# irenemizus/ArtStyleTransfer

Hardware: AMD Instinct MI355X
Metric: style-transfer iters/sec at L=2 (1024-px) (higher is better)
Workload: dtype f32 via f16x2 split (3 f16 MFMAs per product, f32 accumulate; the 14 large-channel conv launches of a closure as Winograd F(2,3) in that arithmetic); 1 GPU; pyramid style transfer, levels_num=3 (1536x1024+768x512+384x256), lbfgs as the reference constructs it (max_eval 1 under torch 2.10), content+noise init, seeded synthetic VGG19 weights, per-step image yield on; parallelism=1 GPU

## Files before the change

artstyletransfer_amd/_lib.py:

```python
from __future__ import annotations

import ctypes as C
import os
import subprocess
import threading

_HERE = os.path.dirname(os.path.abspath(__file__))
LIB_PATH = os.environ.get("NST_LIB") or os.path.join(_HERE, "libnst_hip.so")
CSRC = os.path.join(_HERE, "csrc")

NST_OK = 0
NST_E_STATE = -2
NST_E_UNAVAILABLE = -5
NST_VGG19_CONVS = 13
NST_MAX_LEVELS = 8
NST_LOSS_ROW = 4
NST_OPT_ADAM = 0
NST_OPT_LBFGS = 1
NST_COLOR_RGB = 0
NST_COLOR_LUMINANCE = 1
NST_POOL_MAX = 0
NST_POOL_AVG = 1

c_float_p = C.POINTER(C.c_float)
REDUCE_HOOK = C.CFUNCTYPE(None, C.c_void_p)
c_void = C.c_void_p


NST_CONV_F32, NST_CONV_BF16X3, NST_CONV_F16X2 = 0, 1, 2
CONV_MODES = {"f32": NST_CONV_F32, "bf16x3": NST_CONV_BF16X3, "f16x2": NST_CONV_F16X2}
NST_COMM_ID_BYTES = 128


class StepInfo(C.Structure):
    _fields_ = [("closures", C.c_int), ("total_closures", C.c_int), ("accepted", C.c_int),
                ("loss", C.c_float), ("lr", C.c_float), ("t", C.c_float), ("history", C.c_int)]


class Options(C.Structure):
    _fields_ = [("struct_size", C.c_int), ("conv_mode", C.c_int), ("batched", C.c_int), ("single_stream", C.c_int),
                ("use_graph", C.c_int), ("h2_band_rows", C.c_int), ("lbfgs_gram", C.c_int), ("h2_mfma16", C.c_int),
                ("h2_wg256", C.c_int), ("h2_tile_rows", C.c_int), ("gram_overlap", C.c_int), ("h2_persist", C.c_int), ("level_split", C.c_int), ("h2_winograd", C.c_int)]


SYMBOLS = {
    "nst_version": (C.c_int, []),
    "nst_last_error": (C.c_char_p, [c_void]),
    "nst_device_count": (C.c_int, [C.POINTER(C.c_int)]),
    "nst_ctx_create": (C.c_int, [C.c_int, C.POINTER(c_void), C.POINTER(c_void), C.POINTER(c_void)]),
    "nst_options_default": (None, [C.POINTER(Options)]),
    "nst_ctx_create_ex": (C.c_int, [C.c_int, C.POINTER(c_void), C.POINTER(c_void), C.POINTER(Options), C.POINTER(c_void)]),
    "nst_ctx_destroy": (None, [c_void]),
    "nst_job_configure": (C.c_int, [c_void, C.c_int, C.c_int, C.c_int]),
    "nst_job_set_taps": (C.c_int, [c_void, C.c_int, C.c_uint, C.c_int]),
    "nst_job_set_color": (C.c_int, [c_void, C.c_int]),
    "nst_job_color": (C.c_int, [c_void]),
    "nst_job_set_pooling": (C.c_int, [c_void, C.c_int]),
    "nst_job_pooling": (C.c_int, [c_void]),
    "nst_color_stats": (C.c_int, [c_void, c_void, C.c_int, C.c_int, C.POINTER(C.c_double), C.POINTER(C.c_double), c_void]),
    "nst_color_transfer_matrix": (C.c_int, [C.POINTER(C.c_double)] * 6),
    "nst_color_affine": (C.c_int, [c_void, c_void, C.c_int, C.c_int, C.POINTER(C.c_double), C.POINTER(C.c_double), c_void, c_void]),
    "nst_luminance": (C.c_int, [c_void, c_void, C.c_int, C.c_int, C.c_double, C.c_double, c_void, c_void]),
    "nst_luminance_recombine": (C.c_int, [c_void, c_void, c_void, C.c_int, C.c_int, c_void, c_void]),
    "nst_level_set_targets": (C.c_int, [c_void, C.c_int, c_void, c_void, C.c_int, C.c_int, c_void]),
    "nst_closure": (C.c_int, [c_void, c_void, C.c_float, C.c_float, C.c_float, c_void, c_void, c_void]),
    "nst_closure_levels": (C.c_int, [c_void, c_void, C.c_float, C.c_float, C.c_float, C.c_uint, c_void, c_void, c_void]),
    "nst_closure_forward": (C.c_int, [c_void, c_void, C.c_float, C.c_float, C.c_float, C.c_uint, c_void, c_void]),
    "nst_closure_backward": (C.c_int, [c_void, c_void, C.c_float, C.c_float, C.c_float, C.c_uint, c_void, c_void]),
    "nst_opt_shard_levels": (C.c_int, [c_void, C.c_uint, c_void, c_void, c_void, c_void]),
    "nst_opt_shard_levels_comm": (C.c_int, [c_void, C.c_uint, c_void]),
    "nst_opt_history": (C.c_int, [c_void, C.POINTER(C.c_int), C.POINTER(C.c_int)]),
    "nst_opt_set_closure_reuse": (C.c_int, [c_void, C.c_int]),
    "nst_opt_closure_stats": (C.c_int, [c_void, C.POINTER(C.c_long), C.POINTER(C.c_long)]),
    "nst_opt_set_lazy_backward": (C.c_int, [c_void, C.c_int]),
    "nst_opt_backward_stats": (C.c_int, [c_void, C.POINTER(C.c_long), C.POINTER(C.c_long)]),
    "nst_comm_unique_id": (C.c_int, [c_void]),
    "nst_comm_create": (C.c_int, [C.c_int, C.c_int, C.c_int, c_void, C.POINTER(c_void)]),
    "nst_comm_destroy": (None, [c_void]),
    "nst_comm_info": (C.c_int, [c_void, C.POINTER(C.c_int), C.POINTER(C.c_int), C.POINTER(C.c_long), C.POINTER(C.c_double)]),
    "nst_comm_allreduce_sum": (C.c_int, [c_void, c_void, C.c_size_t, c_void]),
    "nst_adam_step": (C.c_int, [c_void, c_void, c_void, c_void, c_void, C.c_size_t, C.c_int, C.c_double, c_void]),
    "nst_lbfgs_direction": (C.c_int, [c_void, c_void, C.POINTER(c_void), C.POINTER(c_void), C.POINTER(C.c_float), C.c_int,
                                      C.c_float, C.c_size_t, C.c_int, c_void, c_void]),
    "nst_opt_create": (C.c_int, [c_void, C.c_int, C.c_float, C.c_int, C.POINTER(c_void)]),
    "nst_opt_destroy": (None, [c_void]),
    "nst_opt_step": (C.c_int, [c_void, c_void, C.c_float, C.c_float, C.c_float, c_void, C.c_int,
                               C.POINTER(StepInfo), c_void]),
    "nst_vgg_features": (C.c_int, [c_void, c_void, C.c_int, C.c_int, C.POINTER(c_void), c_void]),
    "nst_vgg_features_backward": (C.c_int, [c_void, c_void, C.c_int, C.c_int, C.POINTER(c_void), c_void, c_void]),
    "nst_vgg_activations": (C.c_int, [c_void, c_void, C.c_int, C.c_int, C.POINTER(c_void), c_void]),
    "nst_level_activation": (C.c_int, [c_void, C.c_int, C.c_int, c_void, c_void]),
    "nst_level_image": (C.c_int, [c_void, C.c_int, c_void, c_void]),
    "nst_gram": (C.c_int, [c_void, c_void, C.c_int, C.c_int, C.c_int, C.c_int, c_void, c_void]),
    "nst_total_variation": (C.c_int, [c_void, c_void, C.c_int, C.c_int, C.c_int, c_void, c_void, c_void]),
    "nst_bicubic_half": (C.c_int, [c_void, c_void, C.c_int, C.c_int, C.c_int, c_void, c_void]),
    "nst_bicubic_half_backward": (C.c_int, [c_void, c_void, C.c_int, C.c_int, C.c_int, c_void, c_void]),
    "nst_prepare_img": (C.c_int, [c_void, c_void, C.c_int, C.c_int, c_void, c_void]),
    "nst_unprepare_img": (C.c_int, [c_void, c_void, C.c_int, C.c_int, c_void, c_void]),
    "nst_resize_bicubic": (C.c_int, [c_void, c_void, C.c_int, C.c_int, C.c_int, c_void, C.c_int, C.c_int, c_void]),
    "nst_gather_rows": (C.c_int, [c_void, c_void, c_void, C.c_size_t, C.c_int, c_void, c_void]),
    "nst_gaussian_mask_accumulate": (C.c_int, [c_void, c_void, c_void, C.c_int, C.c_int, C.c_int, C.c_double, C.c_double,
                                               C.c_double, c_void]),
    "nst_noise_blend": (C.c_int, [c_void, c_void, c_void, C.c_int, C.c_int, C.c_int, C.c_double, c_void, c_void]),
    "nst_scale": (C.c_int, [c_void, c_void, C.c_float, C.c_size_t, c_void, c_void]),
    "nst_window_sums_count": (C.c_int, [C.POINTER(C.c_size_t)]),
    "nst_window_begin": (C.c_int, [c_void, c_void, C.c_int, C.c_int, C.c_int, c_void, c_void]),
    "nst_window_end": (C.c_int, [c_void, c_void, C.c_int, C.c_int, C.c_int, C.c_float, C.c_float, C.c_float, c_void, c_void,
                                 c_void, c_void]),
    "nst_conv_mode": (C.c_int, [c_void]),
    "nst_ctx_bytes": (C.c_int, [c_void, C.POINTER(C.c_size_t)]),
    "nst_set_timing": (C.c_int, [c_void, C.c_int]),
    "nst_last_closure_ms": (C.c_int, [c_void, C.POINTER(C.c_float)]),
    "nst_last_closure_class": (C.c_int, [c_void, C.c_int, C.POINTER(C.c_float), C.POINTER(C.c_int),
                                         C.POINTER(C.c_double)]),
    "nst_dump_last_closure": (C.c_int, [c_void]),
    "nst_timing_totals": (C.c_int, [c_void, C.c_int, C.POINTER(C.c_double), C.POINTER(C.c_long),
                                    C.POINTER(C.c_double), C.c_int]),
    "nst_timing_mfma_flops": (C.c_int, [c_void, C.c_int, C.POINTER(C.c_double)]),
}

_lib = None
_lock = threading.Lock()


class NstError(RuntimeError):
    pass


# ... 37 lines not shown
```

artstyletransfer_amd/csrc/nst_opt.cpp:

```cpp
#include <hip/hip_runtime.h>

#include <algorithm>
#include <cmath>
#include <cstdlib>
#include <cstring>
#include <string>
#include <vector>

#include "../../include/nst_hip.h"
#include "nst_kernels.h"

using namespace nst;

extern "C" int nst_internal_device(const nst_ctx* ctx);
extern "C" int nst_internal_levels(const nst_ctx* ctx);
extern "C" size_t nst_internal_pixels(const nst_ctx* ctx);
extern "C" int nst_internal_channels(const nst_ctx* ctx);
extern "C" int nst_internal_fail(nst_ctx* ctx, int code, const char* msg);
extern "C" void nst_internal_poison(void* p, size_t bytes);
extern "C" int nst_internal_zero_now(void* p, size_t bytes);
extern "C" int nst_internal_lbfgs_gram(const nst_ctx* ctx);
extern "C" void nst_internal_mark(nst_ctx* ctx, void* stream);
extern "C" unsigned long long nst_internal_closure_epoch(const nst_ctx* ctx);

// ... 13 lines not shown
    int kind = 0;
    size_t n = 0;
    int channels = 3;
    int levels = 0;
    double lr = 10.0;
    int total_closures = 0;
    float* g = nullptr;
    float* losses = nullptr;
    double* scratch = nullptr;
    float* scal = nullptr;
    float* al_dev = nullptr;
    bool gram_mode = false;
    const float** vec_dev = nullptr;
    float* coef_dev = nullptr;
    double* md_scratch = nullptr;
    float* md_out = nullptr;
    unsigned char* pin2 = nullptr;
    std::vector<double> SY, YY;
    float* pinned = nullptr;
    float* m = nullptr; float* v = nullptr; int k = 0;
    int max_eval = 1;
    int history = 100;
    int n_iter = 0;
    float* d = nullptr; float* prev_g = nullptr; float* xinit = nullptr; float* q = nullptr;
    std::vector<float*> old_dirs, old_stps;
    std::vector<float> ro;
    std::vector<float*> spare;
    float* pool = nullptr;
    hipEvent_t tail = nullptr;
    hipStream_t tail_stream = nullptr;
    bool tail_set = false;
    bool want_rows = false;
    bool H_is_one = true; float H_diag = 1.f;
    bool t_is_float = true;
    double t = 0.0;
    bool have_prev = false;
    unsigned level_mask = 0xFFFFFFFFu;
    nst_reduce_hook hook = nullptr;
    void* hook_user = nullptr;
    float* own_g = nullptr; float* own_losses = nullptr;
    nst_comm* comm = nullptr;
    float* pack = nullptr;
    size_t pack_floats = 0;
    std::vector<float> loss_rows;
    bool reuse = true;
    ClosureMemo memo;
    long served = 0;
    bool lazy = true;
    bool fwd_pending = false;
    bool no_halves = false;
    unsigned long long no_halves_epoch = 0;
    long forward_only = 0;
    long skipped = 0;
};

namespace {

#define OHIP(o, expr)                                                                                \
    do {                                                                                             \
        hipError_t _e = (expr);                                                                      \
        if (_e != hipSuccess)                                                                        \
            return nst_internal_fail((o)->ctx, NST_E_HIP, (std::string(#expr) + ": " + hipGetErrorString(_e)).c_str()); \
    } while (0)
#define OCHK(expr)                   \
    do {                             \
        int _r = (expr);             \
        if (_r != NST_OK) return _r; \
    } while (0)

int oalloc(nst_opt* o, float** p, size_t n) {
    hipError_t e = hipMalloc(reinterpret_cast<void**>(p), n * sizeof(float));
    if (e != hipSuccess) return nst_internal_fail(o->ctx, NST_E_NOMEM, "hipMalloc failed in optimiser");
    nst_internal_poison(*p, n * sizeof(float));
    return NST_OK;
}

struct GradStats {
    bool want_abs = false;
    const float* dot_with = nullptr;
    float gmax = 0.f, gsum = 0.f, gdot = 0.f;
};

int eval_closure(nst_opt* o, const float* x, float cw, float sw, float tvw, hipStream_t s, float* loss_out,
                 GradStats* gs = nullptr, bool forward_only = false) {
    o->lr *= 0.999;
    o->fwd_pending = false;
    if (forward_only && !(o->no_halves && o->no_halves_epoch == nst_internal_closure_epoch(o->ctx))) {
        const int rc = nst_closure_forward(o->ctx, x, cw, sw, tvw, o->level_mask, o->losses, s);
        if (rc == NST_OK) { o->fwd_pending = true; o->forward_only += 1; }
        else if (rc != NST_E_UNAVAILABLE) return rc;
        o->no_halves = rc == NST_E_UNAVAILABLE;
        o->no_halves_epoch = nst_internal_closure_epoch(o->ctx);
    }
    if (!o->fwd_pending) OCHK(nst_closure_levels(o->ctx, x, cw, sw, tvw, o->level_mask, o->g, o->losses, s));
    if (o->comm) OCHK(nst_comm_allreduce_sum(o->comm, o->pack, o->pack_floats, s));
    else if (o->hook) o->hook(o->hook_user);
    const size_t row = (size_t)NST_LOSS_ROW * o->levels + 1;
    const size_t off = o->loss_rows.size();
    o->loss_rows.resize(off + row);
    float* hrow = o->pinned + 8;
    OHIP(o, hipMemcpyAsync(hrow, o->losses, row * sizeof(float), hipMemcpyDeviceToHost, s));
    float* r = o->pinned;
    if (gs && gs->want_abs) OHIP(o, launch_absmax_abssum(o->g, o->n, o->scratch, o->scal, s));
    if (gs && gs->dot_with) OHIP(o, launch_dot(o->g, gs->dot_with, o->n, o->scratch, o->scal + 2, s));
    if (gs) OHIP(o, hipMemcpyAsync(r, o->scal, 3 * sizeof(float), hipMemcpyDeviceToHost, s));
    OHIP(o, hipStreamSynchronize(s));
    if (o->comm) {
        float total = hrow[0];
        for (int l = 1; l < o->levels; ++l) total = total + hrow[(size_t)NST_LOSS_ROW * l];
        hrow[row - 1] = total;
    }
    std::memcpy(o->loss_rows.data() + off, hrow, row * sizeof(float));
    if (gs) { gs->gmax = r[0]; gs->gsum = r[1]; gs->gdot = r[2]; }
    o->total_closures += 1;
    *loss_out = o->loss_rows[off + row - 1];
    return NST_OK;
}

int dot(nst_opt* o, const float* a, const float* b, hipStream_t s, float* out) {
    OHIP(o, launch_dot(a, b, o->n, o->scratch, o->scal, s));
    OHIP(o, hipMemcpyAsync(o->pinned, o->scal, sizeof(float), hipMemcpyDeviceToHost, s));
    OHIP(o, hipStreamSynchronize(s));
    *out = o->pinned[0];
    return NST_OK;
}
int dot2(nst_opt* o, const float* a0, const float* b0, const float* a1, const float* b1, hipStream_t s, float* out0,
         float* out1) {
    float* r = o->pinned;
    OHIP(o, launch_dot(a0, b0, o->n, o->scratch, o->scal, s));
    OHIP(o, launch_dot(a1, b1, o->n, o->scratch, o->scal + 1, s));
    OHIP(o, hipMemcpyAsync(r, o->scal, 2 * sizeof(float), hipMemcpyDeviceToHost, s));
    OHIP(o, hipStreamSynchronize(s));
    *out0 = r[0]; *out1 = r[1];
    return NST_OK;
}
int dot_and_absstats(nst_opt* o, const float* g, const float* d, hipStream_t s, float* gtd, float* mx, float* sum) {
    float* r = o->pinned;
    OHIP(o, launch_absmax_abssum(d, o->n, o->scratch, o->scal, s));
    OHIP(o, launch_dot(g, d, o->n, o->scratch, o->scal + 2, s));
    OHIP(o, hipMemcpyAsync(r, o->scal, 3 * sizeof(float), hipMemcpyDeviceToHost, s));
    OHIP(o, hipStreamSynchronize(s));
    *mx = r[0]; *sum = r[1]; *gtd = r[2];
    return NST_OK;
}
int absstats(nst_opt* o, const float* a, hipStream_t s, float* mx, float* sum) {
    float* r = o->pinned;
    OHIP(o, launch_absmax_abssum(a, o->n, o->scratch, o->scal, s));
    OHIP(o, hipMemcpyAsync(r, o->scal, 2 * sizeof(float), hipMemcpyDeviceToHost, s));
    OHIP(o, hipStreamSynchronize(s));
    *mx = r[0]; *sum = r[1];
    return NST_OK;
}

double cubic_interpolate(double x1, double f1, double g1, double x2, double f2, double g2, bool has_bounds,
                         double lo, double hi) {
    double xmin = has_bounds ? lo : std::min(x1, x2);
    double xmax = has_bounds ? hi : std::max(x1, x2);
    const double d1 = g1 + g2 - 3 * (f1 - f2) / (x1 - x2);
    const double d2sq = d1 * d1 - g1 * g2;
    if (d2sq >= 0) {
        const double d2 = std::sqrt(d2sq);
        double min_pos;
        if (x1 <= x2) min_pos = x2 - (x2 - x1) * ((g2 + d2 - d1) / (g2 - g1 + 2 * d2));
        else min_pos = x1 - (x1 - x2) * ((g1 + d2 - d1) / (g1 - g2 + 2 * d2));
        return std::min(std::max(min_pos, xmin), xmax);
    }
    return (xmin + xmax) / 2.0;
}

struct LsResult { double t; float f; int evals; double last_t; };

bool lazy_applies(const nst_opt* o);

int strong_wolfe(nst_opt* o, float* x, double t, float f, float gtd, float d_norm, int max_ls, float cw, float sw,
                 float tvw, hipStream_t s, LsResult* res) {
    const double c1 = 1e-4, c2 = 0.9, tol_change = 1e-9;
    double last_t = t;
    const bool lazy = lazy_applies(o);
    auto eval_at = [&](double tt, int ls_after, float* f_new, float* gtd_new) -> int {
        last_t = tt;
        OHIP(o, launch_add_scaled(o->xinit, (float)tt, o->d, x, o->n, s));
        if (lazy && ls_after == max_ls) {
            *gtd_new = 0.f;
            return eval_closure(o, x, cw, sw, tvw, s, f_new, nullptr, true);
        }
        GradStats gs;
        gs.dot_with = o->d;
        OCHK(eval_closure(o, x, cw, sw, tvw, s, f_new, &gs));
        *gtd_new = gs.gdot;
        return NST_OK;
    };
    float f_new, gtd_new;
    OCHK(eval_at(t, 0, &f_new, &gtd_new));
    int evals = 1;
    double t_prev = 0; float f_prev = f; float gtd_prev = gtd;
    bool done = false;
    int ls_iter = 0;
    double br[2] = {0, 0}; float br_f[2] = {0, 0}; float br_gtd[2] = {0, 0};
    int nbr = 0;
    while (ls_iter < max_ls) {
        if (f_new > (float)(f + (float)(c1 * t) * gtd) || (ls_iter > 1 && f_new >= f_prev)) {
            br[0] = t_prev; br[1] = t; br_f[0] = f_prev; br_f[1] = f_new; br_gtd[0] = gtd_prev; br_gtd[1] = gtd_new; nbr = 2;
            break;
        }
        if (std::fabs(gtd_new) <= -(float)c2 * gtd) {
            br[0] = t; br_f[0] = f_new; br_gtd[0] = gtd_new; nbr = 1; done = true;
            break;
        }
        if (gtd_new >= 0) {
            br[0] = t_prev; br[1] = t; br_f[0] = f_prev; br_f[1] = f_new; br_gtd[0] = gtd_prev; br_gtd[1] = gtd_new; nbr = 2;
            break;
        }
        const double min_step = t + 0.01 * (t - t_prev);
        const double max_step = t * 10;
        const double tmp = t;
        t = cubic_interpolate(t_prev, f_prev, gtd_prev, t, f_new, gtd_new, true, min_step, max_step);
        t_prev = tmp; f_prev = f_new; gtd_prev = gtd_new;
        OCHK(eval_at(t, ls_iter + 1, &f_new, &gtd_new));
        evals += 1;
        ls_iter += 1;
    }
    if (ls_iter == max_ls && nbr == 0) {
        br[0] = 0; br[1] = t; br_f[0] = f; br_f[1] = f_new; br_gtd[0] = gtd; br_gtd[1] = gtd_new; nbr = 2;
    }
    bool insuf = false;
    int low = (br_f[0] <= br_f[nbr - 1]) ? 0 : 1, high = 1 - low;
    if (nbr == 1) { low = 0; high = 0; }
    while (!done && ls_iter < max_ls) {
        if (std::fabs(br[1] - br[0]) * d_norm < tol_change) break;
        t = cubic_interpolate(br[0], br_f[0], br_gtd[0], br[1], br_f[1], br_gtd[1], false, 0, 0);
        const double bmax = std::max(br[0], br[1]), bmin = std::min(br[0], br[1]);
        const double eps = 0.1 * (bmax - bmin);
        if (std::min(bmax - t, t - bmin) < eps) {
            if (insuf || t >= bmax || t <= bmin) {
                t = (std::fabs(t - bmax) < std::fabs(t - bmin)) ? bmax - eps : bmin + eps;
                insuf = false;
            } else {
                insuf = true;
            }
        } else {
            insuf = false;
        }
        OCHK(eval_at(t, ls_iter + 1, &f_new, &gtd_new));
        evals += 1;
        ls_iter += 1;
        if (f_new > (float)(f + (float)(c1 * t) * gtd) || f_new >= br_f[low]) {
// ... 27 lines not shown
        for (int j = 0; j < i; ++j) v += (al[j] - be[j]) * SYm[(size_t)j * ld + i];
        be[i] = (double)ro[i] * v;
    }
    for (int j = 0; j < m; ++j) { coef[j] = (float)(-(double)Hd * al[j]); coef[m + j] = (float)(al[j] - be[j]); }
}

int gram_direction(nst_opt* o, bool new_pair, hipStream_t s) {
    const int m = (int)o->old_dirs.size();
    const int Hh = o->history;
    const float Hd = o->H_is_one ? 1.f : o->H_diag;
    OHIP(o, launch_scale_copy(-1.f, o->g, o->q, o->n, s));
    if (m == 0) {
        OHIP(o, launch_scale_copy(Hd, o->q, o->d, o->n, s));
        return NST_OK;
    }
    const float** hp = reinterpret_cast<const float**>(o->pin2);
    float* hcoef = reinterpret_cast<float*>(o->pin2 + 2 * (size_t)Hh * sizeof(float*));
    float* hres = hcoef + 2 * (size_t)Hh;
    for (int j = 0; j < m; ++j) { hp[j] = o->old_dirs[j]; hp[m + j] = o->old_stps[j]; }
    OHIP(o, hipMemcpyAsync(o->vec_dev, hp, 2 * (size_t)m * sizeof(float*), hipMemcpyHostToDevice, s));
    const float* a = new_pair ? o->old_stps[m - 1] : o->q;
    const float* b = new_pair ? o->old_dirs[m - 1] : o->q;
    OHIP(o, launch_multi_dot(o->vec_dev, 2 * m, a, b, o->q, o->n, o->md_scratch, o->md_out, s));
    OHIP(o, hipMemcpyAsync(hres, o->md_out, 2 * (size_t)m * 3 * sizeof(float), hipMemcpyDeviceToHost, s));
    OHIP(o, hipStreamSynchronize(s));
    auto SY = [&](int i, int j) -> double& { return o->SY[(size_t)i * Hh + j]; };
    auto YY = [&](int i, int j) -> double& { return o->YY[(size_t)i * Hh + j]; };
    if (new_pair) {
        const int k = m - 1;
        for (int j = 0; j < m; ++j) {
            SY(k, j) = hres[(size_t)j * 3 + 0];
            YY(k, j) = YY(j, k) = hres[(size_t)j * 3 + 1];
            SY(j, k) = hres[(size_t)(m + j) * 3 + 1];
        }
    }
    std::vector<double> sq(m), yq(m);
    for (int i = 0; i < m; ++i) { sq[i] = hres[(size_t)(m + i) * 3 + 2]; yq[i] = hres[(size_t)i * 3 + 2]; }
    direction_coefficients(m, Hh, o->SY.data(), o->YY.data(), o->ro.data(), Hd, sq.data(), yq.data(), hcoef);
    OHIP(o, hipMemcpyAsync(o->coef_dev, hcoef, 2 * (size_t)m * sizeof(float), hipMemcpyHostToDevice, s));
    OHIP(o, launch_multi_axpy(o->vec_dev, o->coef_dev, 2 * m, o->q, Hd, o->d, o->n, s));
    return NST_OK;
}

bool memo_applies(const nst_opt* o) {
    const unsigned all = o->levels >= 32 ? 0xFFFFFFFFu : (1u << o->levels) - 1u;
    return o->reuse && !o->comm && !o->hook && (o->level_mask & all) == all;
}

bool lazy_applies(const nst_opt* o) {
    const unsigned all = o->levels >= 32 ? 0xFFFFFFFFu : (1u << o->levels) - 1u;
    return o->lazy && o->kind == NST_OPT_LBFGS && !o->comm && !o->hook && (o->level_mask & all) == all;
}

int serve_closure(nst_opt* o, const float* x, float cw, float sw, float tvw, unsigned long long epoch, hipStream_t s,
                  bool* served) {
    *served = false;
    ClosureMemo& M = o->memo;
    const float w[3] = {cw, sw, tvw};
    if (std::memcmp(M.w, w, sizeof(w)) != 0 || M.epoch != epoch) return NST_OK;
    float* r = o->pinned;
    OHIP(o, launch_count_diff(x, o->xinit, o->n, o->scratch, o->scal + 3, s));
    if (!M.have_abs) OHIP(o, launch_absmax_abssum(o->g, o->n, o->scratch, o->scal, s));
    OHIP(o, hipMemcpyAsync(r, o->scal, 4 * sizeof(float), hipMemcpyDeviceToHost, s));
    OHIP(o, hipStreamSynchronize(s));
    unsigned diff;
    std::memcpy(&diff, r + 3, sizeof(diff));
    if (diff != 0) return NST_OK;
    if (!M.have_abs) { M.gmax = r[0]; M.gsum = r[1]; M.have_abs = true; }
    o->lr *= 0.999;
    o->loss_rows.insert(o->loss_rows.end(), M.row.begin(), M.row.end());
    o->total_closures += 1;
    o->served += 1;
    *served = true;
    return NST_OK;
}

int form_direction(nst_opt* o, double lr, float gsum, hipStream_t s, double* t, float* gtd, float* d_norm, float* d_sum) {
    if (o->n_iter == 1) {
        OHIP(o, launch_scale_copy(-1.f, o->g, o->d, o->n, s));
        for (float* p : o->old_dirs) o->spare.push_back(p);
        for (float* p : o->old_stps) o->spare.push_back(p);
        o->old_dirs.clear(); o->old_stps.clear(); o->ro.clear();
        o->H_is_one = true; o->H_diag = 1.f;
        if (o->gram_mode) { std::fill(o->SY.begin(), o->SY.end(), 0.0); std::fill(o->YY.begin(), o->YY.end(), 0.0); }
    } else {
        float* y; float* st;
        auto take = [&](float** p) -> int {
            if (o->spare.empty()) return nst_internal_fail(o->ctx, NST_E_STATE, "L-BFGS history pool exhausted");
            *p = o->spare.back(); o->spare.pop_back();
            return NST_OK;
        };
        OCHK(take(&y)); OCHK(take(&st));
        OHIP(o, launch_sub(o->g, o->prev_g, y, o->n, s));
        OHIP(o, launch_scale_copy((float)o->t, o->d, st, o->n, s));
        float ys, yy;
        OCHK(dot2(o, y, st, y, y, s, &ys, &yy));
        bool new_pair = false;
        if (ys > 1e-10f) {
            if ((int)o->old_dirs.size() == o->history) {
                o->spare.push_back(o->old_dirs.front()); o->spare.push_back(o->old_stps.front());
                o->old_dirs.erase(o->old_dirs.begin()); o->old_stps.erase(o->old_stps.begin()); o->ro.erase(o->ro.begin());
                if (o->gram_mode) {
                    const int Hh = o->history;
                    for (int i = 0; i + 1 < Hh; ++i)
                        for (int j = 0; j + 1 < Hh; ++j) {
                            o->SY[(size_t)i * Hh + j] = o->SY[(size_t)(i + 1) * Hh + j + 1];
                            o->YY[(size_t)i * Hh + j] = o->YY[(size_t)(i + 1) * Hh + j + 1];
                        }
                }
            }
            o->old_dirs.push_back(y); o->old_stps.push_back(st); o->ro.push_back(1.0f / ys);
            o->H_diag = ys / yy; o->H_is_one = false;
            new_pair = true;
        } else {
            o->spare.push_back(y); o->spare.push_back(st);
        }
        if (o->gram_mode) {
            OCHK(gram_direction(o, new_pair, s));
        } else {
        const int num_old = (int)o->old_dirs.size();
        double* pp[2] = {o->scratch, o->scratch + RED_BLOCKS};
        int cur = 0;
        OHIP(o, launch_scale_copy(-1.f, o->g, o->q, o->n, s));
        if (num_old > 0) OHIP(o, launch_dot_partial(o->old_stps[num_old - 1], o->q, o->n, pp[cur], s));
        for (int i = num_old - 1; i >= 0; --i) {
            OHIP(o, launch_lbfgs_pair(pp[cur], o->ro[i], o->al_dev + i, 0, o->old_dirs[i], o->q,
                                      i > 0 ? o->old_stps[i - 1] : nullptr, o->n, pp[cur ^ 1], s));
            cur ^= 1;
        }
        OHIP(o, launch_scale_copy(o->H_is_one ? 1.f : o->H_diag, o->q, o->d, o->n, s));
        if (num_old > 0) OHIP(o, launch_dot_partial(o->old_dirs[0], o->d, o->n, pp[cur], s));
        for (int i = 0; i < num_old; ++i) {
            OHIP(o, launch_lbfgs_pair(pp[cur], o->ro[i], o->al_dev + i, 1, o->old_stps[i], o->d,
                                      i + 1 < num_old ? o->old_dirs[i + 1] : nullptr, o->n, pp[cur ^ 1], s));
            cur ^= 1;
        }
        }
    }
    OHIP(o, launch_copy(o->g, o->prev_g, o->n, s));
    o->have_prev = true;
    if (o->n_iter == 1) {
        const float inv = 1.0f / gsum;
        *t = (inv < 1.0f) ? (double)(inv * (float)lr) : lr;
    } else {
        *t = lr;
    }
    OCHK(dot_and_absstats(o, o->g, o->d, s, gtd, d_norm, d_sum));
    return NST_OK;
}

int lbfgs_step(nst_opt* o, float* x, float cw, float sw, float tvw, hipStream_t s, nst_step_info* info) {
    const double lr = o->lr;
    const bool memo_on = memo_applies(o);
    const unsigned long long epoch = nst_internal_closure_epoch(o->ctx);
    ClosureMemo& M = o->memo;
    const bool memo_valid = M.valid;
    M.valid = false;
    bool served = false;
    if (memo_on && memo_valid) OCHK(serve_closure(o, x, cw, sw, tvw, epoch, s, &served));
    const bool reuse_dir = served && M.have_dir;
    float loss, gmax, gsum;
    if (served) {
        loss = M.row.back(); gmax = M.gmax; gsum = M.gsum;
    } else {
        GradStats g0;
        g0.want_abs = true;
        OCHK(eval_closure(o, x, cw, sw, tvw, s, &loss, &g0));
        gmax = g0.gmax; gsum = g0.gsum;
    }
    info->loss = loss;
    const size_t row = (size_t)NST_LOSS_ROW * o->levels + 1;
    auto remember = [&](bool have_dir, bool have_abs, const float* prow, bool copy_x) -> int {
        if (copy_x) OHIP(o, launch_copy(x, o->xinit, o->n, s));
        M.have_dir = have_dir; M.have_abs = have_abs;
        M.gmax = gmax; M.gsum = gsum;
        M.w[0] = cw; M.w[1] = sw; M.w[2] = tvw;
        M.epoch = epoch;
        M.row.assign(prow, prow + row);
        M.valid = true;
        return NST_OK;
    };
    if (gmax <= 1e-7f) {
        info->accepted = 0; info->t = 0.f;
        if (memo_on) OCHK(remember(false, true, o->loss_rows.data(), !served));
        return NST_OK;
    }
    o->n_iter += 1;
    double t;
    float gtd, d_norm, d_sum;
    if (reuse_dir) {
        gtd = M.gtd; d_norm = M.d_norm; d_sum = M.d_sum;
        t = lr;
    } else {
        OCHK(form_direction(o, lr, gsum, s, &t, &gtd, &d_norm, &d_sum));
    }
    info->accepted = 0; info->t = 0.f;
    const bool ran_ls = !(gtd > -1e-9f);
    bool moved = false, g_at_x = false;
    if (ran_ls) {
        if (!served) OHIP(o, launch_copy(x, o->xinit, o->n, s));
        LsResult r;
        OCHK(strong_wolfe(o, x, t, loss, gtd, d_norm, o->max_eval - 1, cw, sw, tvw, s, &r));
        t = r.t;
        if (t != 0.0) OHIP(o, launch_add_scaled(o->xinit, (float)t, o->d, x, o->n, s));
        else OHIP(o, launch_copy(o->xinit, x, o->n, s));
        info->accepted = (t != 0.0) ? 1 : 0;
        info->t = (float)t;
        moved = t != 0.0;
        g_at_x = moved && r.last_t == t;
        if (o->fwd_pending) {
            if (g_at_x) OCHK(nst_closure_backward(o->ctx, x, cw, sw, tvw, o->level_mask, o->g, s));
            else o->skipped += 1;
            o->fwd_pending = false;
        }
    }
    o->t = t;
    if (memo_on) {
        if (!moved) {
            M.gtd = gtd; M.d_norm = d_norm; M.d_sum = d_sum;
            OCHK(remember(true, true, o->loss_rows.data(), !served && !ran_ls));
        } else if (g_at_x) {
            OCHK(remember(false, false, o->loss_rows.data() + o->loss_rows.size() - row, true));
        }
    }
    return NST_OK;
}

}

extern "C" {

int nst_opt_create(nst_ctx* ctx, int kind, float lr_start, int lbfgs_max_eval, nst_opt** out) {
    if (!ctx || !out) return nst_internal_fail(ctx, NST_E_ARG, "null argument");
    if (kind != NST_OPT_ADAM && kind != NST_OPT_LBFGS) return nst_internal_fail(ctx, NST_E_ARG, "Unknown optimizer");
    if (nst_internal_levels(ctx) < 1) return nst_internal_fail(ctx, NST_E_STATE, "nst_job_configure has not been called");
    if (hipSetDevice(nst_internal_device(ctx)) != hipSuccess) return nst_internal_fail(ctx, NST_E_HIP, "hipSetDevice failed");
    nst_opt* o = new (std::nothrow) nst_opt();
    if (!o) return nst_internal_fail(ctx, NST_E_NOMEM, "out of host memory");
    o->ctx = ctx; o->kind = kind; o->lr = (double)lr_start;
    o->levels = nst_internal_levels(ctx);
    o->channels = nst_internal_channels(ctx);
    o->n = (size_t)o->channels * nst_internal_pixels(ctx);
    o->max_eval = lbfgs_max_eval < 1 ? 1 : lbfgs_max_eval;
    const char* reuse_env = std::getenv("NST_CLOSURE_REUSE");
    o->reuse = !(reuse_env && reuse_env[0] && std::atoi(reuse_env) == 0);
    const char* lazy_env = std::getenv("NST_LAZY_BACKWARD");
    o->lazy = !(lazy_env && lazy_env[0] && std::atoi(lazy_env) == 0);
    const size_t row = (size_t)NST_LOSS_ROW * o->levels + 1;
    const size_t n_pad = (o->n + 63) & ~(size_t)63;
    o->pack_floats = n_pad + row;
    int r = oalloc(o, &o->pack, o->pack_floats);
    if (r == NST_OK && nst_internal_zero_now(o->pack, o->pack_floats * sizeof(float))) r = NST_E_HIP;
    o->g = o->own_g = o->pack;
    o->losses = o->own_losses = o->pack ? o->pack + n_pad : nullptr;
    if (r == NST_OK) r = oalloc(o, &o->scal, 4);
    if (r == NST_OK && hipEventCreateWithFlags(&o->tail, hipEventDisableTiming) != hipSuccess) r = NST_E_HIP;
    if (r == NST_OK && kind == NST_OPT_LBFGS) r = oalloc(o, &o->al_dev, (size_t)o->history);
    if (r == NST_OK && kind == NST_OPT_LBFGS && nst_internal_lbfgs_gram(ctx)) {
        const size_t H2 = 2 * (size_t)o->history;
        o->gram_mode = true;
        o->SY.assign((size_t)o->history * o->history, 0.0);
        o->YY.assign((size_t)o->history * o->history, 0.0);
        if (hipMalloc(reinterpret_cast<void**>(&o->vec_dev), H2 * sizeof(float*)) != hipSuccess ||
            hipMalloc(reinterpret_cast<void**>(&o->md_scratch), (size_t)multi_dot_blocks(o->n) * H2 * 3 * sizeof(double)) != hipSuccess ||
            hipHostMalloc(reinterpret_cast<void**>(&o->pin2), H2 * (sizeof(float*) + 4 * sizeof(float)), hipHostMallocDefault) != hipSuccess)
            r = NST_E_NOMEM;
        if (r == NST_OK) r = oalloc(o, &o->coef_dev, H2);
        if (r == NST_OK) r = oalloc(o, &o->md_out, H2 * 3);
    }
    if (r == NST_OK && hipHostMalloc(reinterpret_cast<void**>(&o->pinned), (8 + (size_t)NST_LOSS_ROW * NST_MAX_LEVELS + 1) * sizeof(float), hipHostMallocDefault) != hipSuccess) r = NST_E_NOMEM;
    if (r == NST_OK && hipMalloc(reinterpret_cast<void**>(&o->scratch), 2 * RED_BLOCKS * sizeof(double)) != hipSuccess) r = NST_E_NOMEM;
    if (r == NST_OK && kind == NST_OPT_ADAM) {
        r = oalloc(o, &o->m, o->n);
        if (r == NST_OK) r = oalloc(o, &o->v, o->n);
        if (r == NST_OK && (nst_internal_zero_now(o->m, o->n * 4) || nst_internal_zero_now(o->v, o->n * 4))) r = NST_E_HIP;
    }
    if (r == NST_OK && kind == NST_OPT_LBFGS) {
        r = oalloc(o, &o->d, o->n);
        if (r == NST_OK) r = oalloc(o, &o->prev_g, o->n);
        if (r == NST_OK) r = oalloc(o, &o->xinit, o->n);
        if (r == NST_OK) r = oalloc(o, &o->q, o->n);
        const size_t nvec = 2 * (size_t)o->history + 2;
        if (r == NST_OK) r = oalloc(o, &o->pool, nvec * n_pad);
        if (r == NST_OK) {
            o->spare.reserve(nvec);
            for (size_t i = nvec; i-- > 0;) o->spare.push_back(o->pool + i * n_pad);
        }
    }
    if (r != NST_OK) { nst_opt_destroy(o); return nst_internal_fail(ctx, r, "optimiser allocation failed"); }
    *out = o;
    return NST_OK;
}

void nst_opt_destroy(nst_opt* o) {
    if (!o) return;
    (void)hipSetDevice(nst_internal_device(o->ctx));
    if (o->tail) { (void)hipEventSynchronize(o->tail); (void)hipEventDestroy(o->tail); }
    float* ptrs[] = {o->pack, o->scal, o->al_dev, o->m, o->v, o->d, o->prev_g, o->xinit, o->q, o->pool};
    for (float* p : ptrs) if (p) (void)hipFree(p);
    if (o->scratch) (void)hipFree(o->scratch);
    if (o->pinned) (void)hipHostFree(o->pinned);
    if (o->pin2) (void)hipHostFree(o->pin2);
    if (o->vec_dev) (void)hipFree(o->vec_dev);
    if (o->md_scratch) (void)hipFree(o->md_scratch);
    if (o->coef_dev) (void)hipFree(o->coef_dev);
    if (o->md_out) (void)hipFree(o->md_out);
    delete o;
}

int nst_opt_shard_levels(nst_opt* o, unsigned level_mask, float* grad, float* losses, nst_reduce_hook hook, void* user) {
    if (!o) return nst_internal_fail(nullptr, NST_E_ARG, "null optimiser");
    if ((hook != nullptr) != (grad != nullptr && losses != nullptr))
        return nst_internal_fail(o->ctx, NST_E_ARG, "a reduce hook needs caller-owned grad and losses buffers (and vice versa)");
    o->level_mask = level_mask;
    o->hook = hook; o->hook_user = user;
    o->comm = nullptr;
    o->memo.valid = false;
    o->g = grad ? grad : o->own_g;
    o->losses = losses ? losses : o->own_losses;
    return NST_OK;
}

int nst_opt_shard_levels_comm(nst_opt* o, unsigned level_mask, nst_comm* comm) {
    if (!o) return nst_internal_fail(nullptr, NST_E_ARG, "null optimiser");
    o->level_mask = comm ? level_mask : 0xFFFFFFFFu;
    o->hook = nullptr; o->hook_user = nullptr;
    o->comm = comm;
    o->g = o->own_g; o->losses = o->own_losses;
    o->memo.valid = false;
    return NST_OK;
}

int nst_opt_history(const nst_opt* o, int* pairs, int* n_iter) {
    if (!o) return nst_internal_fail(nullptr, NST_E_ARG, "null optimiser");
    if (pairs) *pairs = (int)o->old_dirs.size();
    if (n_iter) *n_iter = o->kind == NST_OPT_ADAM ? o->k : o->n_iter;
    return NST_OK;
}

int nst_opt_set_closure_reuse(nst_opt* o, int enabled) {
    if (!o) return nst_internal_fail(nullptr, NST_E_ARG, "null optimiser");
    o->reuse = enabled != 0;
    o->memo.valid = false;
    return NST_OK;
}

int nst_opt_closure_stats(const nst_opt* o, long* evaluated, long* served) {
    if (!o) return nst_internal_fail(nullptr, NST_E_ARG, "null optimiser");
    if (evaluated) *evaluated = (long)o->total_closures - o->served;
    if (served) *served = o->served;
    return NST_OK;
}

int nst_opt_set_lazy_backward(nst_opt* o, int enabled) {
    if (!o) return nst_internal_fail(nullptr, NST_E_ARG, "null optimiser");
    o->lazy = enabled != 0;
    return NST_OK;
}

int nst_opt_backward_stats(const nst_opt* o, long* forward_only, long* skipped) {
    if (!o) return nst_internal_fail(nullptr, NST_E_ARG, "null optimiser");
    if (forward_only) *forward_only = o->forward_only;
    if (skipped) *skipped = o->skipped;
    return NST_OK;
}

static int adam_update(nst_ctx* ctx, float* x, const float* g, float* m, float* v, size_t n, int k, double lr, hipStream_t s,
                       float* step_size_out) {
    const double bc1 = 1.0 - std::pow(0.9, k);
    const double bc2 = 1.0 - std::pow(0.999, k);
    const double step_size = lr / bc1;
    const hipError_t e = launch_adam(x, g, m, v, n, 0.999f, (float)(1.0 - 0.9), (float)(1.0 - 0.999), 1e-8f, (float)step_size,
                                     (float)std::sqrt(bc2), s);
    if (e != hipSuccess) return nst_internal_fail(ctx, NST_E_HIP, hipGetErrorString(e));
    if (step_size_out) *step_size_out = (float)step_size;
    return NST_OK;
}

int nst_adam_step(nst_ctx* ctx, float* x, const float* g, float* m, float* v, size_t n, int k, double lr, void* stream) {
    if (!ctx || !x || !g || !m || !v || k < 1) return nst_internal_fail(ctx, NST_E_ARG, "bad argument");
    if (hipSetDevice(nst_internal_device(ctx)) != hipSuccess) return nst_internal_fail(ctx, NST_E_HIP, "hipSetDevice failed");
    return adam_update(ctx, x, g, m, v, n, k, lr, static_cast<hipStream_t>(stream), nullptr);
}

int nst_lbfgs_direction(nst_ctx* ctx, const float* g, const float* const* y, const float* const* sv, const float* ro, int m,
                        float h_diag, size_t n, int form, float* d, void* stream) {
    if (!ctx || !g || !d || m < 0 || (m > 0 && (!y || !sv || !ro)) || (form != 0 && form != 1))
        return nst_internal_fail(ctx, NST_E_ARG, "bad argument");
    if (hipSetDevice(nst_internal_device(ctx)) != hipSuccess) return nst_internal_fail(ctx, NST_E_HIP, "hipSetDevice failed");
    hipStream_t s = static_cast<hipStream_t>(stream);
    nst_opt tmp;
    tmp.ctx = ctx;
    nst_opt* o = &tmp;
    float* q = nullptr; float* al_dev = nullptr; float* coef_dev = nullptr; float* md_out = nullptr;
    double* scratch = nullptr; double* md_scratch = nullptr; const float** vec_dev = nullptr;
    auto cleanup = [&]() {
        (void)hipStreamSynchronize(s);
        for (void* p : {(void*)q, (void*)al_dev, (void*)coef_dev, (void*)md_out, (void*)scratch, (void*)md_scratch, (void*)vec_dev})
            if (p) (void)hipFree(p);
    };
    auto body = [&]() -> int {
        OHIP(o, hipMalloc(reinterpret_cast<void**>(&q), n * sizeof(float)));
        OHIP(o, launch_scale_copy(-1.f, g, q, n, s));
        if (m == 0) { OHIP(o, launch_scale_copy(h_diag, q, d, n, s)); return NST_OK; }
        if (form == 1) {
            OHIP(o, hipMalloc(reinterpret_cast<void**>(&al_dev), (size_t)m * sizeof(float)));
            OHIP(o, hipMalloc(reinterpret_cast<void**>(&scratch), 2 * RED_BLOCKS * sizeof(double)));
            double* pp[2] = {scratch, scratch + RED_BLOCKS};
            int cur = 0;
// ... 96 lines not shown
```

artstyletransfer_amd/engine.py:

```python
from __future__ import annotations

import ctypes as C
from typing import List, Optional, Sequence, Tuple

import numpy as np
import torch

from . import _lib
from . import taps as _taps
from .pooling_modes import check_pooling
from ._lib import NST_LOSS_ROW, NstError, StepInfo

TAP_CHANNELS = (64, 128, 256, 512, 512, 512)
TAP_SCALE = (0, 1, 2, 3, 3, 4)
DEFAULT_TAPS = (_taps.DEFAULT_CONTENT_INDEX, _taps.DEFAULT_STYLE_INDICES, True)


def _ptr(t: Optional[torch.Tensor]):
    return C.c_void_p(t.data_ptr()) if t is not None else C.c_void_p(0)


def _stream(device) -> C.c_void_p:
    return C.c_void_p(torch.cuda.current_stream(device).cuda_stream)

# ... 466 lines not shown

class PixelOptimizer:

    def __init__(self, engine: StyleEngine, name: str, lr_start: float = 10.0, lbfgs_max_eval: int = 1):
        if name == "adam":
            kind = _lib.NST_OPT_ADAM
        elif name == "lbfgs":
            kind = _lib.NST_OPT_LBFGS
        else:
            raise RuntimeError("Unknown optimizer")
        self.engine = engine
        self.name = name
        h = C.c_void_p()
        _lib.check(engine.ctx, engine.lib.nst_opt_create(engine.ctx, kind, lr_start, lbfgs_max_eval, C.byref(h)),
                   "nst_opt_create")
        self.h = h
        self.channels = engine.channels
        self.row = NST_LOSS_ROW * engine.levels + 1
        self.cap = 32 if name == "lbfgs" else 1
        self._rows = np.zeros((self.cap, self.row), dtype=np.float32)

    def shard_levels_comm(self, comm: "Communicator") -> None:
        from . import sharding
        e = self.engine
        self._comm = comm
        _lib.check(e.ctx, e.lib.nst_opt_shard_levels_comm(self.h, sharding.level_mask(e.levels, comm.rank, comm.world),
                                                          comm.h), "nst_opt_shard_levels_comm")

    def history(self):
        p, n = C.c_int(), C.c_int()
        _lib.check(self.engine.ctx, self.engine.lib.nst_opt_history(self.h, C.byref(p), C.byref(n)), "nst_opt_history")
        return p.value, n.value

    def set_closure_reuse(self, enabled: bool) -> None:
        _lib.check(self.engine.ctx, self.engine.lib.nst_opt_set_closure_reuse(self.h, int(bool(enabled))),
                   "nst_opt_set_closure_reuse")

    def closure_stats(self):
        ev, sv = C.c_long(), C.c_long()
        _lib.check(self.engine.ctx, self.engine.lib.nst_opt_closure_stats(self.h, C.byref(ev), C.byref(sv)),
                   "nst_opt_closure_stats")
        return ev.value, sv.value

    def set_lazy_backward(self, enabled: bool) -> None:
        _lib.check(self.engine.ctx, self.engine.lib.nst_opt_set_lazy_backward(self.h, int(bool(enabled))),
                   "nst_opt_set_lazy_backward")

    def backward_stats(self):
        fo, sk = C.c_long(), C.c_long()
        _lib.check(self.engine.ctx, self.engine.lib.nst_opt_backward_stats(self.h, C.byref(fo), C.byref(sk)),
                   "nst_opt_backward_stats")
        return fo.value, sk.value

    def shard_levels(self, rank: int, world: int, dist_mod=None, group=None) -> None:
        from . import sharding
        e = self.engine
        H, W = e.shape
        self._g = torch.zeros((1, self.channels, H, W), dtype=torch.float32, device=e.device)
        self._l = torch.zeros(self.row, dtype=torch.float32, device=e.device)

        def hook(_user):
            sharding.allreduce_closure(self._g, self._l, dist_mod, group)

        self._hook = _lib.REDUCE_HOOK(hook)
        _lib.check(e.ctx, e.lib.nst_opt_shard_levels(self.h, sharding.level_mask(e.levels, rank, world),
                                                     _ptr(self._g), _ptr(self._l), self._hook, None),
                   "nst_opt_shard_levels")

    def shard_stripes(self, rank: int, world: int, weights, content_t, style_t,
                      dist_mod=None, group=None, comm: "Communicator" = None) -> None:
        from . import sharding
        if comm is not None:
            rank, world = comm.rank, comm.world
        elif dist_mod is None:
            import torch.distributed as dist_mod
        contents = list(content_t) if isinstance(content_t, (list, tuple)) else [content_t]
        styles = list(style_t) if isinstance(style_t, (list, tuple)) else [style_t]
        e = self.engine
        if e.channels != 3:
            raise NstError("the stripe closure implements RGB only (set_color('rgb'))")
        H, W = e.shape
        nstriped = min(len(contents), len(styles), e.levels)
        plans, stripes = [], []
        for l in range(nstriped):
            plan = sharding.StripePlan(H >> l, world, rank)
            st = StyleEngine(weights, e.device)
            st.configure(1, plan.ext_rows, W >> l)
            st.set_targets(0, plan.cut(contents[l]), styles[l].contiguous())
            plans.append(plan)
            stripes.append(st)
        self._stripes, self._plans = stripes, plans
        self._stripe, self._plan = stripes[0], plans[0]
        n = 3 * H * W
        self._pack = torch.zeros(n + self.row, dtype=torch.float32, device=e.device)
        self._g = self._pack[:n].view(1, 3, H, W)
        self._l = self._pack[n:]
        count = stripes[0].window_sums_count()
        sums_all = torch.empty(nstriped * count, dtype=torch.float32, device=e.device)
        mask = 0
        for l in sharding.deal_levels(range(nstriped, e.levels), world)[rank]:
            mask |= 1 << l

        def hook(_user):
            x, (cw, sw, tvw) = self._x, self._w
            imgs, cuts = [x], []
            for l in range(nstriped):
# ... 97 lines not shown
```

include/nst_hip.h:

```cpp
#ifndef NST_HIP_H
#define NST_HIP_H

#include <stddef.h>
#include <stdint.h>

#ifdef __cplusplus
extern "C" {
#endif

#define NST_OK 0
#define NST_E_ARG (-1)
#define NST_E_STATE (-2)
#define NST_E_HIP (-3)
#define NST_E_NOMEM (-4)
#define NST_E_UNAVAILABLE (-5)

#define NST_VGG19_CONVS 13
#define NST_MAX_LEVELS 8
#define NST_LOSS_ROW 4

typedef struct nst_ctx nst_ctx;
typedef struct nst_opt nst_opt;
typedef struct nst_comm nst_comm;

// ... 37 lines not shown
int nst_job_color(const nst_ctx* ctx);

#define NST_POOL_MAX 0
#define NST_POOL_AVG 1
int nst_job_set_pooling(nst_ctx* ctx, int mode);
int nst_job_pooling(const nst_ctx* ctx);

int nst_level_set_targets(nst_ctx* ctx, int level, const float* content, const float* style,
                          int hs, int ws, void* stream);

int nst_closure(nst_ctx* ctx, const float* x, float content_weight, float style_weight,
                float tv_weight, float* grad, float* losses, void* stream);

int nst_closure_levels(nst_ctx* ctx, const float* x, float content_weight, float style_weight,
                       float tv_weight, unsigned level_mask, float* grad, float* losses, void* stream);

int nst_closure_forward(nst_ctx* ctx, const float* x, float content_weight, float style_weight, float tv_weight,
                        unsigned level_mask, float* losses, void* stream);
int nst_closure_backward(nst_ctx* ctx, const float* x, float content_weight, float style_weight, float tv_weight,
                         unsigned level_mask, float* grad, void* stream);

#define NST_OPT_ADAM 0
#define NST_OPT_LBFGS 1
int nst_opt_create(nst_ctx* ctx, int kind, float lr_start, int lbfgs_max_eval, nst_opt** out);
void nst_opt_destroy(nst_opt* opt);

typedef struct nst_step_info {
    int closures;
    int total_closures;
    int accepted;
    float loss;
    float lr;
    float t;
    int history;
} nst_step_info;

int nst_opt_step(nst_opt* opt, float* x, float content_weight, float style_weight, float tv_weight,
                 float* losses_host, int closures_capacity, nst_step_info* info, void* stream);

typedef void (*nst_reduce_hook)(void* user);
int nst_opt_shard_levels(nst_opt* opt, unsigned level_mask, float* grad, float* losses, nst_reduce_hook hook,
                         void* user);

int nst_opt_shard_levels_comm(nst_opt* opt, unsigned level_mask, nst_comm* comm);

int nst_opt_history(const nst_opt* opt, int* pairs, int* n_iter);

int nst_opt_set_closure_reuse(nst_opt* opt, int enabled);
int nst_opt_closure_stats(const nst_opt* opt, long* evaluated, long* served);

int nst_opt_set_lazy_backward(nst_opt* opt, int enabled);
int nst_opt_backward_stats(const nst_opt* opt, long* forward_only, long* skipped);

#define NST_COMM_ID_BYTES 128
int nst_comm_unique_id(void* id);
int nst_comm_create(int device, int rank, int world, const void* id, nst_comm** out);
void nst_comm_destroy(nst_comm* comm);
int nst_comm_info(const nst_comm* comm, int* rank, int* world, long* calls, double* bytes);
int nst_comm_allreduce_sum(nst_comm* comm, float* buf, size_t n, void* stream);

int nst_adam_step(nst_ctx* ctx, float* x, const float* g, float* m, float* v, size_t n, int k, double lr, void* stream);
int nst_lbfgs_direction(nst_ctx* ctx, const float* g, const float* const* y, const float* const* s, const float* ro, int m,
                        float h_diag, size_t n, int form, float* d, void* stream);


int nst_vgg_features(nst_ctx* ctx, const float* x, int h, int w, float* const* outs, void* stream);
int nst_vgg_activations(nst_ctx* ctx, const float* x, int h, int w, float* const* outs, void* stream);
int nst_vgg_features_backward(nst_ctx* ctx, const float* x, int h, int w, const float* const* gouts,
                              float* gx, void* stream);
int nst_level_activation(nst_ctx* ctx, int level, int layer, float* out, void* stream);
int nst_level_image(nst_ctx* ctx, int level, float* out, void* stream);
int nst_gram(nst_ctx* ctx, const float* f, int C, int h, int w, int normalize, float* gram, void* stream);
int nst_total_variation(nst_ctx* ctx, const float* y, int C, int h, int w, float* value, float* grad,
                        void* stream);
int nst_bicubic_half(nst_ctx* ctx, const float* x, int C, int h, int w, float* y, void* stream);
int nst_bicubic_half_backward(nst_ctx* ctx, const float* gy, int C, int h, int w, float* gx, void* stream);
int nst_prepare_img(nst_ctx* ctx, const float* hwc, int h, int w, float* chw, void* stream);
int nst_unprepare_img(nst_ctx* ctx, const float* chw, int h, int w, float* hwc, void* stream);


int nst_resize_bicubic(nst_ctx* ctx, const float* src, int h, int w, int channels, float* dst, int nh, int nw, void* stream);
int nst_gather_rows(nst_ctx* ctx, const float* src, const long long* perm, size_t rows, int channels, float* dst, void* stream);
int nst_gaussian_mask_accumulate(nst_ctx* ctx, float* acc, const float* src, int h, int w, int channels, double central,
                                 double peripheral, double dispersion, void* stream);
int nst_noise_blend(nst_ctx* ctx, const float* content, const float* noise, int h, int w, int channels, double noise_factor,
                    float* out, void* stream);
int nst_scale(nst_ctx* ctx, const float* src, float alpha, size_t n, float* dst, void* stream);

int nst_color_stats(nst_ctx* ctx, const float* hwc, int h, int w, double* mean, double* cov, void* stream);
int nst_color_transfer_matrix(const double* mean_c, const double* cov_c, const double* mean_s, const double* cov_s, double* A,
                              double* b);
int nst_color_affine(nst_ctx* ctx, const float* src, int h, int w, const double* A, const double* b, float* dst, void* stream);
int nst_luminance(nst_ctx* ctx, const float* hwc, int h, int w, double alpha, double beta, float* out, void* stream);
int nst_luminance_recombine(nst_ctx* ctx, const float* u, const float* content, int h, int w, float* out, void* stream);

int nst_window_sums_count(size_t* count);
int nst_window_begin(nst_ctx* ctx, const float* xs, int row0, int rows, int H0, float* sums, void* stream);
int nst_window_end(nst_ctx* ctx, const float* xs, int row0, int rows, int H0, float content_weight, float style_weight,
                   float tv_weight, float* sums, float* gxs, float* losses, void* stream);

int nst_conv_mode(const nst_ctx* ctx);

int nst_ctx_bytes(const nst_ctx* ctx, size_t* bytes);

int nst_set_timing(nst_ctx* ctx, int enabled);
int nst_last_closure_ms(nst_ctx* ctx, float* ms);
// ... 10 lines not shown
```

Before: 445.8 iters/s.

## Speculatively evaluate the L-BFGS trial point before confirming closure memo equality

When the closure memo applies and max_eval is 1, the optimiser launches the forward pass at xinit + lr*d straight away, together with the equality check against the incoming x. It then reads back the losses and the diff flag in one synchronisation. If the inputs match, the memoised closure and the trial forward are both booked, and the line search reuses that loss instead of evaluating again. The intent is to remove a separate host sync and readback between serving the memo and the trial forward. If the check fails, the speculative forward is wasted work, and the bookkeeping of lr and loss rows becomes more intricate.

```diff
diff --git a/artstyletransfer_amd/_lib.py b/artstyletransfer_amd/_lib.py
--- a/artstyletransfer_amd/_lib.py
+++ b/artstyletransfer_amd/_lib.py
@@ -74,6 +74,8 @@
     "nst_opt_closure_stats": (C.c_int, [c_void, C.POINTER(C.c_long), C.POINTER(C.c_long)]),
     "nst_opt_set_lazy_backward": (C.c_int, [c_void, C.c_int]),
     "nst_opt_backward_stats": (C.c_int, [c_void, C.POINTER(C.c_long), C.POINTER(C.c_long)]),
+    "nst_opt_set_trial_speculation": (C.c_int, [c_void, C.c_int]),
+    "nst_opt_speculation_stats": (C.c_int, [c_void, C.POINTER(C.c_long), C.POINTER(C.c_long)]),
     "nst_comm_unique_id": (C.c_int, [c_void]),
     "nst_comm_create": (C.c_int, [C.c_int, C.c_int, C.c_int, c_void, C.POINTER(c_void)]),
     "nst_comm_destroy": (None, [c_void]),
diff --git a/artstyletransfer_amd/csrc/nst_opt.cpp b/artstyletransfer_amd/csrc/nst_opt.cpp
--- a/artstyletransfer_amd/csrc/nst_opt.cpp
+++ b/artstyletransfer_amd/csrc/nst_opt.cpp
@@ -89,6 +89,9 @@
     unsigned long long no_halves_epoch = 0;
     long forward_only = 0;
     long skipped = 0;
+    bool speculate = true;
+    long spec_launched = 0;
+    long spec_discarded = 0;
 };
 
 namespace {
@@ -118,6 +121,13 @@
     float gmax = 0.f, gsum = 0.f, gdot = 0.f;
 };
 
+void book_row(nst_opt* o, const float* hrow, float* loss_out) {
+    const size_t row = (size_t)NST_LOSS_ROW * o->levels + 1;
+    o->loss_rows.insert(o->loss_rows.end(), hrow, hrow + row);
+    o->total_closures += 1;
+    *loss_out = o->loss_rows.back();
+}
+
 int eval_closure(nst_opt* o, const float* x, float cw, float sw, float tvw, hipStream_t s, float* loss_out,
                  GradStats* gs = nullptr, bool forward_only = false) {
     o->lr *= 0.999;
@@ -133,8 +143,6 @@
     if (o->comm) OCHK(nst_comm_allreduce_sum(o->comm, o->pack, o->pack_floats, s));
     else if (o->hook) o->hook(o->hook_user);
     const size_t row = (size_t)NST_LOSS_ROW * o->levels + 1;
-    const size_t off = o->loss_rows.size();
-    o->loss_rows.resize(off + row);
     float* hrow = o->pinned + 8;
     OHIP(o, hipMemcpyAsync(hrow, o->losses, row * sizeof(float), hipMemcpyDeviceToHost, s));
     float* r = o->pinned;
@@ -147,10 +155,8 @@
         for (int l = 1; l < o->levels; ++l) total = total + hrow[(size_t)NST_LOSS_ROW * l];
         hrow[row - 1] = total;
     }
-    std::memcpy(o->loss_rows.data() + off, hrow, row * sizeof(float));
     if (gs) { gs->gmax = r[0]; gs->gsum = r[1]; gs->gdot = r[2]; }
-    o->total_closures += 1;
-    *loss_out = o->loss_rows[off + row - 1];
+    book_row(o, hrow, loss_out);
     return NST_OK;
 }
 
@@ -210,7 +216,7 @@
 bool lazy_applies(const nst_opt* o);
 
 int strong_wolfe(nst_opt* o, float* x, double t, float f, float gtd, float d_norm, int max_ls, float cw, float sw,
-                 float tvw, hipStream_t s, LsResult* res) {
+                 float tvw, hipStream_t s, LsResult* res, const float* pre_f = nullptr) {
     const double c1 = 1e-4, c2 = 0.9, tol_change = 1e-9;
     double last_t = t;
     const bool lazy = lazy_applies(o);
@@ -228,7 +234,8 @@
         return NST_OK;
     };
     float f_new, gtd_new;
-    OCHK(eval_at(t, 0, &f_new, &gtd_new));
+    if (pre_f) { f_new = *pre_f; gtd_new = 0.f; }
+    else OCHK(eval_at(t, 0, &f_new, &gtd_new));
     int evals = 1;
     double t_prev = 0; float f_prev = f; float gtd_prev = gtd;
     bool done = false;
@@ -362,6 +369,13 @@
     return o->lazy && o->kind == NST_OPT_LBFGS && !o->comm && !o->hook && (o->level_mask & all) == all;
 }
 
+void book_served(nst_opt* o) {
+    o->lr *= 0.999;
+    o->loss_rows.insert(o->loss_rows.end(), o->memo.row.begin(), o->memo.row.end());
+    o->total_closures += 1;
+    o->served += 1;
+}
+
 int serve_closure(nst_opt* o, const float* x, float cw, float sw, float tvw, unsigned long long epoch, hipStream_t s,
                   bool* served) {
     *served = false;
@@ -377,11 +391,41 @@
     std::memcpy(&diff, r + 3, sizeof(diff));
     if (diff != 0) return NST_OK;
     if (!M.have_abs) { M.gmax = r[0]; M.gsum = r[1]; M.have_abs = true; }
+    book_served(o);
+    *served = true;
+    return NST_OK;
+}
+
+bool speculation_applies(const nst_opt* o, float cw, float sw, float tvw, unsigned long long epoch) {
+    const ClosureMemo& M = o->memo;
+    const float w[3] = {cw, sw, tvw};
+    return o->speculate && lazy_applies(o) && o->max_eval - 1 == 0 && M.have_dir && M.have_abs &&
+           std::memcmp(M.w, w, sizeof(w)) == 0 && M.epoch == epoch && M.gmax > 1e-7f && !(M.gtd > -1e-9f) &&
+           !(o->no_halves && o->no_halves_epoch == epoch);
+}
+int speculative_trial(nst_opt* o, const float* x, double t, float cw, float sw, float tvw, unsigned long long epoch,
+                      hipStream_t s, bool* launched, bool* equal, float* f_trial) {
+    *launched = false; *equal = false;
+    const size_t row = (size_t)NST_LOSS_ROW * o->levels + 1;
+    OHIP(o, launch_add_scaled(o->xinit, (float)t, o->d, o->q, o->n, s));
+    const int rc = nst_closure_forward(o->ctx, o->q, cw, sw, tvw, o->level_mask, o->losses, s);
+    if (rc == NST_E_UNAVAILABLE) { o->no_halves = true; o->no_halves_epoch = epoch; return NST_OK; }
+    OCHK(rc);
+    *launched = true;
+    o->spec_launched += 1;
+    OHIP(o, launch_count_diff(x, o->xinit, o->n, o->scratch, o->losses + row, s));
+    float* hrow = o->pinned + 8;
+    OHIP(o, hipMemcpyAsync(hrow, o->losses, (row + 1) * sizeof(float), hipMemcpyDeviceToHost, s));
+    OHIP(o, hipStreamSynchronize(s));
+    unsigned diff;
+    std::memcpy(&diff, hrow + row, sizeof(diff));
+    if (diff != 0) { o->spec_discarded += 1; return NST_OK; }
+    *equal = true;
+    book_served(o);
     o->lr *= 0.999;
-    o->loss_rows.insert(o->loss_rows.end(), M.row.begin(), M.row.end());
-    o->total_closures += 1;
-    o->served += 1;
-    *served = true;
+    o->fwd_pending = true;
+    o->forward_only += 1;
+    book_row(o, hrow, f_trial);
     return NST_OK;
 }
 
@@ -467,7 +511,13 @@
     const bool memo_valid = M.valid;
     M.valid = false;
     bool served = false;
-    if (memo_on && memo_valid) OCHK(serve_closure(o, x, cw, sw, tvw, epoch, s, &served));
+    bool spec = false, spec_launched = false;
+    float spec_f = 0.f;
+    if (memo_on && memo_valid && speculation_applies(o, cw, sw, tvw, epoch)) {
+        OCHK(speculative_trial(o, x, lr, cw, sw, tvw, epoch, s, &spec_launched, &spec, &spec_f));
+        served = spec;
+    }
+    if (memo_on && memo_valid && !spec_launched) OCHK(serve_closure(o, x, cw, sw, tvw, epoch, s, &served));
     const bool reuse_dir = served && M.have_dir;
     float loss, gmax, gsum;
     if (served) {
@@ -510,16 +560,16 @@
     if (ran_ls) {
         if (!served) OHIP(o, launch_copy(x, o->xinit, o->n, s));
         LsResult r;
-        OCHK(strong_wolfe(o, x, t, loss, gtd, d_norm, o->max_eval - 1, cw, sw, tvw, s, &r));
+        OCHK(strong_wolfe(o, x, t, loss, gtd, d_norm, o->max_eval - 1, cw, sw, tvw, s, &r, spec ? &spec_f : nullptr));
         t = r.t;
         if (t != 0.0) OHIP(o, launch_add_scaled(o->xinit, (float)t, o->d, x, o->n, s));
-        else OHIP(o, launch_copy(o->xinit, x, o->n, s));
+        else if (!spec) OHIP(o, launch_copy(o->xinit, x, o->n, s));
         info->accepted = (t != 0.0) ? 1 : 0;
         info->t = (float)t;
         moved = t != 0.0;
         g_at_x = moved && r.last_t == t;
         if (o->fwd_pending) {
-            if (g_at_x) OCHK(nst_closure_backward(o->ctx, x, cw, sw, tvw, o->level_mask, o->g, s));
+            if (g_at_x) OCHK(nst_closure_backward(o->ctx, spec ? o->q : x, cw, sw, tvw, o->level_mask, o->g, s));
             else o->skipped += 1;
             o->fwd_pending = false;
         }
@@ -556,11 +606,13 @@
     o->reuse = !(reuse_env && reuse_env[0] && std::atoi(reuse_env) == 0);
     const char* lazy_env = std::getenv("NST_LAZY_BACKWARD");
     o->lazy = !(lazy_env && lazy_env[0] && std::atoi(lazy_env) == 0);
+    const char* spec_env = std::getenv("NST_TRIAL_SPECULATION");
+    o->speculate = !(spec_env && spec_env[0] && std::atoi(spec_env) == 0);
     const size_t row = (size_t)NST_LOSS_ROW * o->levels + 1;
     const size_t n_pad = (o->n + 63) & ~(size_t)63;
     o->pack_floats = n_pad + row;
-    int r = oalloc(o, &o->pack, o->pack_floats);
-    if (r == NST_OK && nst_internal_zero_now(o->pack, o->pack_floats * sizeof(float))) r = NST_E_HIP;
+    int r = oalloc(o, &o->pack, o->pack_floats + 1);
+    if (r == NST_OK && nst_internal_zero_now(o->pack, (o->pack_floats + 1) * sizeof(float))) r = NST_E_HIP;
     o->g = o->own_g = o->pack;
     o->losses = o->own_losses = o->pack ? o->pack + n_pad : nullptr;
     if (r == NST_OK) r = oalloc(o, &o->scal, 4);
@@ -578,7 +630,7 @@
         if (r == NST_OK) r = oalloc(o, &o->coef_dev, H2);
         if (r == NST_OK) r = oalloc(o, &o->md_out, H2 * 3);
     }
-    if (r == NST_OK && hipHostMalloc(reinterpret_cast<void**>(&o->pinned), (8 + (size_t)NST_LOSS_ROW * NST_MAX_LEVELS + 1) * sizeof(float), hipHostMallocDefault) != hipSuccess) r = NST_E_NOMEM;
+    if (r == NST_OK && hipHostMalloc(reinterpret_cast<void**>(&o->pinned), (8 + (size_t)NST_LOSS_ROW * NST_MAX_LEVELS + 2) * sizeof(float), hipHostMallocDefault) != hipSuccess) r = NST_E_NOMEM;
     if (r == NST_OK && hipMalloc(reinterpret_cast<void**>(&o->scratch), 2 * RED_BLOCKS * sizeof(double)) != hipSuccess) r = NST_E_NOMEM;
     if (r == NST_OK && kind == NST_OPT_ADAM) {
         r = oalloc(o, &o->m, o->n);
@@ -665,6 +717,19 @@
 int nst_opt_set_lazy_backward(nst_opt* o, int enabled) {
     if (!o) return nst_internal_fail(nullptr, NST_E_ARG, "null optimiser");
     o->lazy = enabled != 0;
+    return NST_OK;
+}
+
+int nst_opt_set_trial_speculation(nst_opt* o, int enabled) {
+    if (!o) return nst_internal_fail(nullptr, NST_E_ARG, "null optimiser");
+    o->speculate = enabled != 0;
+    return NST_OK;
+}
+
+int nst_opt_speculation_stats(const nst_opt* o, long* launched, long* discarded) {
+    if (!o) return nst_internal_fail(nullptr, NST_E_ARG, "null optimiser");
+    if (launched) *launched = o->spec_launched;
+    if (discarded) *discarded = o->spec_discarded;
     return NST_OK;
 }
 
diff --git a/artstyletransfer_amd/engine.py b/artstyletransfer_amd/engine.py
--- a/artstyletransfer_amd/engine.py
+++ b/artstyletransfer_amd/engine.py
@@ -542,6 +542,16 @@
                    "nst_opt_backward_stats")
         return fo.value, sk.value
 
+    def set_trial_speculation(self, enabled: bool) -> None:
+        _lib.check(self.engine.ctx, self.engine.lib.nst_opt_set_trial_speculation(self.h, int(bool(enabled))),
+                   "nst_opt_set_trial_speculation")
+
+    def speculation_stats(self):
+        la, di = C.c_long(), C.c_long()
+        _lib.check(self.engine.ctx, self.engine.lib.nst_opt_speculation_stats(self.h, C.byref(la), C.byref(di)),
+                   "nst_opt_speculation_stats")
+        return la.value, di.value
+
     def shard_levels(self, rank: int, world: int, dist_mod=None, group=None) -> None:
         from . import sharding
         e = self.engine
diff --git a/include/nst_hip.h b/include/nst_hip.h
--- a/include/nst_hip.h
+++ b/include/nst_hip.h
@@ -113,6 +113,9 @@
 int nst_opt_set_lazy_backward(nst_opt* opt, int enabled);
 int nst_opt_backward_stats(const nst_opt* opt, long* forward_only, long* skipped);
 
+int nst_opt_set_trial_speculation(nst_opt* opt, int enabled);
+int nst_opt_speculation_stats(const nst_opt* opt, long* launched, long* discarded);
+
 #define NST_COMM_ID_BYTES 128
 int nst_comm_unique_id(void* id);
 int nst_comm_create(int device, int rank, int world, const void* id, nst_comm** out);
```

New measurement: 446.8 iters/s (median of 6 runs). About the same (+0.2%).
